# TMElyralab/MuseV

Hardware: NVIDIA H100
Metric: denoised frames/sec at 512x512, 16-frame window, 20 DDIM steps (higher is better)
Workload: dtype f16 (fp32 accumulate)

## Files before the change

musev_b200/csrc/conv_gemm.cu:

```cuda
#include "conv_gemm.cuh"

#include <dlfcn.h>
#include <stdio.h>
#include <stdlib.h>
#include <string.h>

#include <mutex>

#include "ptx.cuh"
#include "stats.cuh"

namespace mvb {

static constexpr int kMaxStages = 8;
static constexpr int kBlockM = 128;
static constexpr int kBlockK = 64;
static constexpr int kABytes = kBlockM * kBlockK * 2;
static constexpr int kSmemBytes = 227 * 1024;
constexpr bool inline_epilogue(int bn) { return bn == 256; }
constexpr int conv_threads(int bn) { return inline_epilogue(bn) ? 384 : 512; }
static constexpr int kMaxStagedN = 160;
static constexpr int kStagingBytes = kBlockM * kMaxStagedN * 4;
static constexpr int kAccLd = 132;
static constexpr int kAccBytes = 2 * 64 * kAccLd * 4;
constexpr int epi_buf_bytes(int bn) { return inline_epilogue(bn) ? kAccBytes : kStagingBytes; }
constexpr int bias_buf_bytes(int bn) { return inline_epilogue(bn) ? 2 * 256 * 4 : kMaxStagedN * 4; }
constexpr int ring_bytes(int bn) { return kSmemBytes - epi_buf_bytes(bn) - bias_buf_bytes(bn) - 1024  - 256 ; }
constexpr int ring_stage_bytes(int bn) { return kABytes + (bn * kBlockK * 2 + 1023) / 1024 * 1024; }
constexpr int ring_stages(int bn) {
  return ring_bytes(bn) / ring_stage_bytes(bn) < kMaxStages ? ring_bytes(bn) / ring_stage_bytes(bn) : kMaxStages;
}
static_assert(ring_stages(64) == 6 && ring_stages(128) == 4 && ring_stages(160) == 4 && ring_stages(256) == 3,
              "shared-memory budget per tile width");
__device__ __forceinline__ float gelu_erf(float x) { return 0.5f * x * (1.f + erff(x * 0.70710678118654752440f)); }
__device__ __forceinline__ float silu(float x) { return __fdividef(x, 1.f + __expf(-x)); }
__device__ __forceinline__ float gelu_fast(float x) {
  const float z = fabsf(x) * 0.70710678118654752440f;
  const float t = __frcp_rn(fmaf(0.3275911f, z, 1.f));
  float poly = fmaf(1.061405429f, t, -1.453152027f);
  poly = fmaf(poly, t, 1.421413741f);
  poly = fmaf(poly, t, -0.284496736f);
  poly = fmaf(poly, t, 0.254829592f);
  poly *= t;
  float e;
  asm("ex2.approx.ftz.f32 %0, %1;" : "=f"(e) : "f"(-z * z * 1.4426950408889634f));
  const float erf_abs = fmaf(-poly, e, 1.f);
  const float erf_v = copysignf(erf_abs, x);
  return 0.5f * x * (1.f + erf_v);
}

__device__ __forceinline__ float rcp_approx(float x) {
  float y;
  asm("rcp.approx.ftz.f32 %0, %1;" : "=f"(y) : "f"(x));
  return y;
}
__device__ __forceinline__ F2 geglu2(F2 val, F2 gate) {
  float g0, g1;
  f2_get(gate, g0, g1);
  const F2 u = f2_make(fabsf(g0), fabsf(g1));
  float d0, d1;
  f2_get(f2_fma(u, f2_make(0.231641888f, 0.231641888f), f2_make(1.f, 1.f)), d0, d1);
  const F2 t = f2_make(rcp_approx(d0), rcp_approx(d1));
  F2 poly = f2_fma(t, f2_make(-0.5307027145f, -0.5307027145f), f2_make(0.7265760135f, 0.7265760135f));
  poly = f2_fma(poly, t, f2_make(-0.7107068705f, -0.7107068705f));
  poly = f2_fma(poly, t, f2_make(0.142248368f, 0.142248368f));
  poly = f2_fma(poly, t, f2_make(-0.127414796f, -0.127414796f));
  poly = f2_mul(poly, t);
  float a0, a1;
  f2_get(f2_mul(f2_mul(u, f2_make(-0.72134752044f, -0.72134752044f)), u), a0, a1);
  float e0, e1;
  asm("ex2.approx.ftz.f32 %0, %1;" : "=f"(e0) : "f"(a0));
  asm("ex2.approx.ftz.f32 %0, %1;" : "=f"(e1) : "f"(a1));
  const F2 gelu = f2_fma(u, f2_mul(poly, f2_make(e0, e1)), f2_make(fmaxf(g0, 0.f), fmaxf(g1, 0.f)));
  return f2_mul(val, gelu);
}

enum : int {
  kEpiGeneric = 0,
  kEpiPlain = 1,
  kEpiResidual = 2,
  kEpiGeglu = 3,
  kEpiAct = 4
};
__device__ __forceinline__ float gelu_act(float x, int act) {
  return act == 2 ? gelu_erf(x) : act == 3 ? __fdividef(x, 1.f + __expf(-1.702f * x)) : x;
}

struct AMaps {
  CUtensorMap m[4];
};

template <int kEpi, class Ld>
__device__ __forceinline__ void finish_run(const ConvGemmParams& p, const Ld& ld32, int c0, int ncol0, const float* sbias,
                                           const float* radd, const uint4 (&rcur)[4], bool row_ok, bool use_res,
                                           long long m, __half* out_row) {
  if constexpr (kEpi != kEpiGeneric && kEpi != kEpiAct) {
    const int nbase = ncol0 + c0;
    uint32_t v[32], vg[32];
    ld32(c0, v);
    if constexpr (kEpi == kEpiGeglu) ld32(c0 + 32, vg);
    if (nbase < p.N && row_ok) {
      const F2 alpha2 = f2_make(p.alpha, p.alpha);
      const float* cbias = sbias + c0;
      const int oc = (kEpi == kEpiGeglu) ? nbase / 2 : nbase;
#pragma unroll
      for (int g = 0; g < 4; ++g) {
        uint32_t o[4];
        if constexpr (kEpi == kEpiGeglu) {
          const uint32_t* vv = (g < 2) ? v : vg;
          const int j0 = (g & 1) * 8;
#pragma unroll
          for (int e = 0; e < 4; ++e) {
            const int j = j0 + 2 * e;
            const float2 bv = *reinterpret_cast<const float2*>(cbias + (g >> 1) * 32 + j);
            const float2 bg = *reinterpret_cast<const float2*>(cbias + (g >> 1) * 32 + 16 + j);
            const F2 val = f2_add(f2_make(__uint_as_float(vv[j]), __uint_as_float(vv[j + 1])), f2_make(bv.x, bv.y));
            const F2 gat = f2_add(f2_make(__uint_as_float(vv[16 + j]), __uint_as_float(vv[16 + j + 1])),
                                  f2_make(bg.x, bg.y));
            float x0, x1;
            f2_get(geglu2(val, gat), x0, x1);
            const __half2 h2 = __floats2half2_rn(x0, x1);
            o[e] = *reinterpret_cast<const uint32_t*>(&h2);
          }
        } else {
          float4 b0 = *reinterpret_cast<const float4*>(cbias + 8 * g);
          float4 b1 = *reinterpret_cast<const float4*>(cbias + 8 * g + 4);
          if (radd) {
            const float4 a0 = __ldg(reinterpret_cast<const float4*>(radd + nbase) + 2 * g);
            const float4 a1 = __ldg(reinterpret_cast<const float4*>(radd + nbase) + 2 * g + 1);
            b0.x += a0.x; b0.y += a0.y; b0.z += a0.z; b0.w += a0.w;
            b1.x += a1.x; b1.y += a1.y; b1.z += a1.z; b1.w += a1.w;
          }
          const float bb[8] = {b0.x, b0.y, b0.z, b0.w, b1.x, b1.y, b1.z, b1.w};
          const __half2* rh2 = reinterpret_cast<const __half2*>(&rcur[g]);
#pragma unroll
          for (int e = 0; e < 4; ++e) {
            const int j = g * 8 + 2 * e;
            F2 x = f2_add(f2_make(__uint_as_float(v[j]), __uint_as_float(v[j + 1])), f2_make(bb[2 * e], bb[2 * e + 1]));
            if constexpr (kEpi == kEpiResidual) {
              const float2 rr = __half22float2(rh2[e]);
              x = f2_fma(x, alpha2, f2_make(rr.x, rr.y));
            }
            float x0, x1;
            f2_get(x, x0, x1);
            const __half2 h2 = __floats2half2_rn(x0, x1);
            o[e] = *reinterpret_cast<const uint32_t*>(&h2);
          }
        }
        *reinterpret_cast<uint4*>(out_row + oc + 8 * g) = make_uint4(o[0], o[1], o[2], o[3]);
      }
    }
  } else {
    float f[32];
    const int nbase = ncol0 + c0;
    if (p.geglu) {
      uint32_t va[32], vb[32];
      ld32(c0, va);
      ld32(c0 + 32, vb);
#pragma unroll
      for (int hsel = 0; hsel < 2; ++hsel) {
        const uint32_t* v = hsel ? vb : va;
        const int nb = nbase + hsel * 32;
#pragma unroll
        for (int j4 = 0; j4 < 4; ++j4) {
          const bool bok = p.bias && nb < p.N;
          const float4 bv = bok ? __ldg(reinterpret_cast<const float4*>(p.bias + nb) + j4) : make_float4(0, 0, 0, 0);
          const float4 bg = bok ? __ldg(reinterpret_cast<const float4*>(p.bias + nb + 16) + j4) : make_float4(0, 0, 0, 0);
          const int j = j4 * 4;
          const F2 v01 = f2_add(f2_make(__uint_as_float(v[j]), __uint_as_float(v[j + 1])), f2_make(bv.x, bv.y));
          const F2 v23 = f2_add(f2_make(__uint_as_float(v[j + 2]), __uint_as_float(v[j + 3])), f2_make(bv.z, bv.w));
          const F2 g01 = f2_add(f2_make(__uint_as_float(v[16 + j]), __uint_as_float(v[16 + j + 1])), f2_make(bg.x, bg.y));
          const F2 g23 = f2_add(f2_make(__uint_as_float(v[16 + j + 2]), __uint_as_float(v[16 + j + 3])), f2_make(bg.z, bg.w));
          f2_get(geglu2(v01, g01), f[hsel * 16 + j], f[hsel * 16 + j + 1]);
          f2_get(geglu2(v23, g23), f[hsel * 16 + j + 2], f[hsel * 16 + j + 3]);
        }
      }
    } else {
      uint32_t v[32];
      ld32(c0, v);
      if (nbase + 32 <= p.N) {
#pragma unroll
        for (int g = 0; g < 8; ++g) {
          float4 b = p.bias ? __ldg(reinterpret_cast<const float4*>(p.bias + nbase) + g) : make_float4(0, 0, 0, 0);
          if (radd) {
            const float4 a4 = __ldg(reinterpret_cast<const float4*>(radd + nbase) + g);
            b.x += a4.x; b.y += a4.y; b.z += a4.z; b.w += a4.w;
          }
          f[g * 4 + 0] = __uint_as_float(v[g * 4 + 0]) + b.x;
          f[g * 4 + 1] = __uint_as_float(v[g * 4 + 1]) + b.y;
          f[g * 4 + 2] = __uint_as_float(v[g * 4 + 2]) + b.z;
          f[g * 4 + 3] = __uint_as_float(v[g * 4 + 3]) + b.w;
        }
      } else {
#pragma unroll
        for (int j = 0; j < 32; ++j) {
          const int nn = nbase + j;
          float x = __uint_as_float(v[j]);
          if (nn < p.N) {
            if (p.bias) x += __ldg(p.bias + nn);
            if (radd) x += __ldg(radd + nn);
          }
          f[j] = x;
        }
      }
    }
    if (row_ok) {
      if (p.out_f32) {
#pragma unroll
        for (int g = 0; g < 8; ++g) {
          const int nn = nbase + g * 4;
          if (nn < p.N) {
            float4 o4;
            o4.x = f[g * 4 + 0] * p.alpha; o4.y = f[g * 4 + 1] * p.alpha;
            o4.z = f[g * 4 + 2] * p.alpha; o4.w = f[g * 4 + 3] * p.alpha;
            if (p.act == 1) { o4.x = silu(o4.x); o4.y = silu(o4.y); o4.z = silu(o4.z); o4.w = silu(o4.w); }
            if constexpr (kEpi == kEpiAct) {
              o4.x = gelu_act(o4.x, p.act); o4.y = gelu_act(o4.y, p.act);
              o4.z = gelu_act(o4.z, p.act); o4.w = gelu_act(o4.w, p.act);
            }
            *reinterpret_cast<float4*>(reinterpret_cast<float*>(p.out) + m * p.ldc + nn) = o4;
          }
        }
      } else {
        const int oc = p.geglu ? nbase / 2 : nbase;
        const int ncols = p.geglu ? p.N / 2 : p.N;
#pragma unroll
        for (int g = 0; g < 4; ++g) {
          if (oc + 8 * g >= ncols) continue;
          __align__(16) __half o[8];
          const __half* rh8 = reinterpret_cast<const __half*>(&rcur[g]);
#pragma unroll
          for (int j = 0; j < 8; ++j) {
            float x = f[g * 8 + j];
            if (!p.geglu) {
              x *= p.alpha;
              if (use_res) x = fmaf(p.beta, __half2float(rh8[j]), x);
              if (p.act == 1) x = silu(x);
              if constexpr (kEpi == kEpiAct) x = gelu_act(x, p.act);
            }
            o[j] = __float2half_rn(x);
          }
          *reinterpret_cast<uint4*>(out_row + oc + 8 * g) = *reinterpret_cast<const uint4*>(o);
        }
      }
    }
  }
}

template <int kEpi, int BN>
__device__ __forceinline__ void inline_epilogue_tile(const ConvGemmParams& p, const float (&acc)[BN / 2], float* sacc,
                                                     float* sbias, int unit, int wg, int t) {
  const int lane = t & 31;
  const int wq = t >> 5;
  const int row_local = t & 63;
  const int half = t >> 6;
  const int r = 64 * wg + row_local;
  float* acc_slice = sacc + wg * 64 * kAccLd;
  float* wbias = sbias + wg * 256;
  const bool use_res = (p.res != nullptr) && !p.geglu && !p.out_f32;
  const int acc_step = p.geglu ? 64 : 32;
  const int nt = unit % p.tiles_nn;
  const int mt = unit / p.tiles_nn;
  const int tw = mt % p.tiles_w;
  const int th = (mt / p.tiles_w) % p.tiles_h;
  const int tn = mt / (p.tiles_w * p.tiles_h);
  const int ncol0 = nt * BN;
  const int rw = r % p.bw;
  const int rh = (r / p.bw) % p.bh;
  const int rn = r / (p.bw * p.bh);
  const int w = tw * p.bw + rw, h = th * p.bh + rh, n = tn * p.bn + rn;
  const bool row_ok = (w < p.W) && (h < p.H) && (n < p.NF);
  const long long m = ((long long)n * p.H + h) * p.W + w;
  const float* radd = (p.rowadd && row_ok) ? p.rowadd + (long long)(m / p.rows_per_group) * p.ld_rowadd : nullptr;
  const __half* res_row = use_res ? p.res + m * p.ld_res : nullptr;
  __half* out_row = reinterpret_cast<__half*>(p.out) + m * p.ldc;

  uint4 rcur[4] = {};
  auto load_res = [&](int c0) {
    if (!use_res || !row_ok) return;
#pragma unroll
    for (int g = 0; g < 4; ++g) {
      const int nn = ncol0 + c0 + g * 8;
      if (c0 + g * 8 < BN && nn < p.N) rcur[g] = __ldg(reinterpret_cast<const uint4*>(res_row + nn));
    }
  };
  named_bar_sync(1 + wg, 128);
  if constexpr (kEpi != kEpiGeneric && kEpi != kEpiAct) {
    for (int c = t; c < BN; c += 128) wbias[c] = (p.bias && ncol0 + c < p.N) ? __ldg(p.bias + ncol0 + c) : 0.f;
  }
#pragma unroll
  for (int u = 0; u < (BN + 127) / 128; ++u) {
    if (u > 0) named_bar_sync(1 + wg, 128);
#pragma unroll
    for (int i = 16 * u; i < 16 * u + 16 && i < BN / 8; ++i) {
      const int rr = 16 * wq + (lane >> 2);
      const int cc = 8 * (i - 16 * u) + 2 * (lane & 3);
      *reinterpret_cast<float2*>(acc_slice + rr * kAccLd + cc) = make_float2(acc[4 * i], acc[4 * i + 1]);
      *reinterpret_cast<float2*>(acc_slice + (rr + 8) * kAccLd + cc) = make_float2(acc[4 * i + 2], acc[4 * i + 3]);
    }
    named_bar_sync(1 + wg, 128);
    const int cend = (128 * u + 128 < BN) ? 128 * u + 128 : BN;
    for (int c0 = 128 * u + half * acc_step; c0 < cend; c0 += 2 * acc_step) {
      const float* srow = acc_slice + row_local * kAccLd - 128 * u;
      auto ld32 = [&](int col, uint32_t (&v)[32]) {
#pragma unroll
        for (int k = 0; k < 8; ++k) {
          const float4 x = *reinterpret_cast<const float4*>(srow + col + 4 * k);
          v[4 * k] = __float_as_uint(x.x); v[4 * k + 1] = __float_as_uint(x.y);
          v[4 * k + 2] = __float_as_uint(x.z); v[4 * k + 3] = __float_as_uint(x.w);
        }
      };
      load_res(c0);
      finish_run<kEpi>(p, ld32, c0, ncol0, wbias, radd, rcur, row_ok, use_res, m, out_row);
    }
  }
}

template <int kEpi, int BN>
__global__ void __launch_bounds__(conv_threads(BN), 1)
conv_gemm_kernel(const __grid_constant__ AMaps tmA, const __grid_constant__ CUtensorMap tmB,
                 const __grid_constant__ ConvGemmParams p) {
  constexpr bool kInline = inline_epilogue(BN);
  static_assert(BN % 32 == 0 && (BN <= kMaxStagedN || kInline), "the staging swizzle and the epilogue take whole 32-column runs");
  constexpr int kProducerRegs = 40, kConsumerRegs = kInline ? 232 : 152, kEpilogueRegs = kInline ? 0 : 168;
  static_assert(128 * (kProducerRegs + kEpilogueRegs) + 256 * kConsumerRegs <= 65536,
                "setmaxnreg split exceeds the register file");
  constexpr int kRingBytes = ring_bytes(BN);
  extern __shared__ uint8_t smem_raw[];
  uint8_t* smem = reinterpret_cast<uint8_t*>((reinterpret_cast<uintptr_t>(smem_raw) + 1023) & ~uintptr_t(1023));
  float* stg = reinterpret_cast<float*>(smem + kRingBytes);
  float* sbias = reinterpret_cast<float*>(smem + kRingBytes + epi_buf_bytes(BN));
  uint64_t* bars = reinterpret_cast<uint64_t*>(smem + kRingBytes + epi_buf_bytes(BN) + bias_buf_bytes(BN));
  uint64_t* full = bars;
  uint64_t* empty = bars + kMaxStages;
  uint64_t* acc_full = bars + 2 * kMaxStages;
  uint64_t* acc_empty = acc_full + 1;
  const int nstages = p.nstages;
  const int stage_bytes = p.stage_bytes;

  const int warp = threadIdx.x >> 5;
  const int lane = threadIdx.x & 31;

  if (threadIdx.x == 0) {
    tma_prefetch_desc(&tmA.m[0]);
    tma_prefetch_desc(&tmA.m[1]);
    tma_prefetch_desc(&tmA.m[2]);
    tma_prefetch_desc(&tmA.m[3]);
    tma_prefetch_desc(&tmB);
    for (int s = 0; s < kMaxStages; ++s) {
      mbar_init(&full[s], 1);
      mbar_init(&empty[s], 8);
    }
    mbar_init(acc_full, 8);
    mbar_init(acc_empty, 4);
    fence_barrier_init();
  }
  __syncthreads();

  const int kb_per_tap = p.kb0 + p.kb1;
  const int num_kb = p.ntaps * kb_per_tap;
  const int tiles_m = p.tiles_w * p.tiles_h * p.tiles_n;
  const int num_units = tiles_m * p.tiles_nn;
  const uint32_t stage_tx = kABytes + (uint32_t)BN * kBlockK * 2;

  if (warp < 4) {
    setmaxnreg_dec<kProducerRegs>();
    if (warp == 0) {
      int stage = 0;
      uint32_t phase = 0;
      for (int unit = blockIdx.x; unit < num_units; unit += gridDim.x) {
        const int nt = unit % p.tiles_nn;
        const int mt = unit / p.tiles_nn;
        const int tw = mt % p.tiles_w;
        const int th = (mt / p.tiles_w) % p.tiles_h;
        const int tn = mt / (p.tiles_w * p.tiles_h);
        const int w0 = tw * p.bw, h0 = th * p.bh, n0 = tn * p.bn;
        int kcol = 0;
        const int ncoord = nt * BN;
        for (int tap = 0; tap < p.ntaps; ++tap) {
          const int xw = w0 + p.dx[tap], yh = h0 + p.dy[tap];
          const int src0 = p.tap_src[tap];
          for (int cb = 0; cb < kb_per_tap; ++cb, kcol += kBlockK) {
            const bool first = cb < p.kb0;
            const int src = src0 + (first ? 0 : 1);
            const int c0 = (first ? cb : cb - p.kb0) * kBlockK;
            const CUtensorMap* tm = &tmA.m[src];
            mbar_wait(&empty[stage], phase ^ 1);
            if (elect_one()) {
              uint8_t* sa = smem + stage * stage_bytes;
              uint8_t* sb = sa + kABytes;
              mbar_expect_tx(&full[stage], stage_tx);
              tma_load_4d(sa, tm, &full[stage], c0, xw, yh, n0);
              tma_load_2d(sb, &tmB, &full[stage], kcol, ncoord);
            }
            __syncwarp();
            if (++stage == nstages) { stage = 0; phase ^= 1; }
          }
        }
      }
    }
    return;
  }

  if (!kInline && warp >= 12) {
    setmaxnreg_inc<kEpilogueRegs>();
    const int r = threadIdx.x - 384;
    const float* srow = stg + r * BN;
    const int sw = r & 7;
    const bool use_res = (p.res != nullptr) && !p.geglu && !p.out_f32;
    const int acc_step = p.geglu ? 64 : 32;
    uint32_t acc_phase = 0;
    for (int unit = blockIdx.x; unit < num_units; unit += gridDim.x) {
      const int nt = unit % p.tiles_nn;
      const int mt = unit / p.tiles_nn;
      const int tw = mt % p.tiles_w;
      const int th = (mt / p.tiles_w) % p.tiles_h;
      const int tn = mt / (p.tiles_w * p.tiles_h);
      const int ncol0 = nt * BN;
      const int rw = r % p.bw;
      const int rh = (r / p.bw) % p.bh;
      const int rn = r / (p.bw * p.bh);
      const int w = tw * p.bw + rw, h = th * p.bh + rh, n = tn * p.bn + rn;
      const bool row_ok = (w < p.W) && (h < p.H) && (n < p.NF);
      const long long m = ((long long)n * p.H + h) * p.W + w;
      const float* radd = (p.rowadd && row_ok) ? p.rowadd + (long long)(m / p.rows_per_group) * p.ld_rowadd : nullptr;
      const __half* res_row = use_res ? p.res + m * p.ld_res : nullptr;
      __half* out_row = reinterpret_cast<__half*>(p.out) + m * p.ldc;

      uint4 rcur[4] = {}, rnext[4] = {};
      auto load_res = [&](int c0, uint4 (&dst)[4]) {
        if (!use_res || !row_ok) return;
#pragma unroll
        for (int g = 0; g < 4; ++g) {
          const int nn = ncol0 + c0 + g * 8;
          if (c0 + g * 8 < BN && nn < p.N) dst[g] = __ldg(reinterpret_cast<const uint4*>(res_row + nn));
        }
      };
      if constexpr (kEpi != kEpiGeneric && kEpi != kEpiAct) {
        named_bar_sync(1, 128);
        for (int c = r; c < BN; c += 128) sbias[c] = (p.bias && ncol0 + c < p.N) ? __ldg(p.bias + ncol0 + c) : 0.f;
        named_bar_sync(1, 128);
      }
      load_res(0, rcur);
      mbar_wait(acc_full, acc_phase);
      for (int c0 = 0; c0 < BN; c0 += acc_step) {
        if constexpr (kEpi == kEpiResidual) load_res(c0 + acc_step, rnext);
        else if (c0 > 0) load_res(c0, rcur);
        auto ld32 = [&](int col, uint32_t (&v)[32]) {
#pragma unroll
          for (int k = 0; k < 8; ++k) {
            const float4 x = *reinterpret_cast<const float4*>(srow + col + 4 * (k ^ sw));
            v[4 * k] = __float_as_uint(x.x); v[4 * k + 1] = __float_as_uint(x.y);
            v[4 * k + 2] = __float_as_uint(x.z); v[4 * k + 3] = __float_as_uint(x.w);
          }
        };
        finish_run<kEpi>(p, ld32, c0, ncol0, sbias, radd, rcur, row_ok, use_res, m, out_row);
        if constexpr (kEpi == kEpiResidual) {
#pragma unroll
          for (int g = 0; g < 4; ++g) rcur[g] = rnext[g];
        }
      }
      __syncwarp();
      if (lane == 0) mbar_arrive(acc_empty);
      acc_phase ^= 1;
    }
    return;
  }

  setmaxnreg_inc<kConsumerRegs>();
  const int wg = (warp - 4) >> 2;
  const int t = threadIdx.x - 128 * (1 + wg);
  const int wq = t >> 5;
  const uint64_t desc0_a = make_desc_k_sw128(smem_u32(smem) + (uint32_t)wg * 64 * 128);
  const uint64_t desc0_b = make_desc_k_sw128(smem_u32(smem) + kABytes);
  const uint32_t stage_step = (uint32_t)stage_bytes >> 4;
  float* stg_row = stg + (64 * wg + 16 * wq + (lane >> 2)) * BN;
  int stage = 0;
  uint32_t phase = 0;
  uint32_t acc_phase = 0;
  float acc[BN / 2];

  for (int unit = blockIdx.x; unit < num_units; unit += gridDim.x) {
    int prev_stage = 0;
    for (int kb = 0; kb < num_kb; ++kb) {
      mbar_wait(&full[stage], phase);
      const uint64_t da = desc0_a + (uint64_t)((uint32_t)stage * stage_step);
      const uint64_t db = desc0_b + (uint64_t)((uint32_t)stage * stage_step);
      wgmma_fence();
      fence_regs(acc);
#pragma unroll
      for (int k = 0; k < kBlockK / 16; ++k)
        Wgmma<BN>::ss(acc, da + (uint64_t)(k * 2), db + (uint64_t)(k * 2), (kb | k) != 0);
      wgmma_commit();
      fence_regs(acc);
      if (kb > 0) {
        wgmma_wait<1>();
        fence_regs(acc);
        __syncwarp();
        if (lane == 0) mbar_arrive(&empty[prev_stage]);
      }
      prev_stage = stage;
      if (++stage == nstages) { stage = 0; phase ^= 1; }
    }
    wgmma_wait<0>();
    fence_regs(acc);
    __syncwarp();
    if (lane == 0) mbar_arrive(&empty[prev_stage]);

    if constexpr (kInline) {
      inline_epilogue_tile<kEpi, BN>(p, acc, stg, sbias, unit, wg, t);
    } else {
      mbar_wait(acc_empty, acc_phase ^ 1);
#pragma unroll
      for (int i = 0; i < BN / 8; ++i) {
        const int off = 4 * ((2 * i + ((lane & 3) >> 1)) ^ (lane >> 2)) + 2 * (lane & 1);
        *reinterpret_cast<float2*>(stg_row + off) = make_float2(acc[4 * i], acc[4 * i + 1]);
        *reinterpret_cast<float2*>(stg_row + 8 * BN + off) = make_float2(acc[4 * i + 2], acc[4 * i + 3]);
      }
      __syncwarp();
      if (lane == 0) mbar_arrive(acc_full);
      acc_phase ^= 1;
    }
  }
}

typedef CUresult (*EncodeTiledFn)(CUtensorMap*, CUtensorMapDataType, cuuint32_t, void*, const cuuint64_t*,
                                  const cuuint64_t*, const cuuint32_t*, const cuuint32_t*, CUtensorMapInterleave,
                                  CUtensorMapSwizzle, CUtensorMapL2promotion, CUtensorMapFloatOOBfill);

EncodeTiledFn get_encode_fn() {
  static EncodeTiledFn fn = nullptr;
  static bool tried = false;
  if (!tried) {
    tried = true;
    void* h = dlopen("libcuda.so.1", RTLD_NOW | RTLD_GLOBAL);
    if (!h) h = dlopen("libcuda.so", RTLD_NOW | RTLD_GLOBAL);
    if (h) fn = reinterpret_cast<EncodeTiledFn>(dlsym(h, "cuTensorMapEncodeTiled"));
  }
  return fn;
}

namespace {
struct MapKey {
  uint64_t ptr, d[4], s[3];
  uint32_t box[4], rank, swz;
  bool operator==(const MapKey& o) const { return memcmp(this, &o, sizeof(MapKey)) == 0; }
};
struct MapSlot {
  MapKey key;
  CUtensorMap map;
  bool used;
};
static_assert(sizeof(MapKey) == 88, "MapKey is compared and hashed bytewise: no padding allowed");
static_assert(sizeof(MapSlot) % 64 == 0, "slots keep the 64-byte alignment of CUtensorMap");
constexpr uint32_t kMapSlots = 1u << 14;
std::mutex g_map_mutex;
MapSlot* g_map_slots = nullptr;
uint32_t g_map_count = 0;
unsigned long long g_map_hits = 0, g_map_misses = 0;

uint64_t hash_key(const MapKey& k) {
  const uint64_t* w = reinterpret_cast<const uint64_t*>(&k);
  uint64_t h = 0x9e3779b97f4a7c15ull;
  for (size_t i = 0; i < sizeof(MapKey) / 8; ++i) {
    h ^= w[i] + 0x9e3779b97f4a7c15ull + (h << 6) + (h >> 2);
    h *= 0xff51afd7ed558ccdull;
    h ^= h >> 33;
  }
  return h;
}
bool cache_enabled() {
  static const bool on = !(getenv("MVB_TMAP_CACHE") && atoi(getenv("MVB_TMAP_CACHE")) == 0);
  return on;
}

bool encode_raw(CUtensorMap* m, const MapKey& k) {
  EncodeTiledFn fn = get_encode_fn();
  if (!fn) return false;
  cuuint64_t gd[4] = {k.d[0], k.d[1], k.d[2], k.d[3]};
  cuuint64_t gs[3] = {k.s[0] * 2, k.s[1] * 2, k.s[2] * 2};
  cuuint32_t bx[4] = {k.box[0], k.box[1], k.box[2], k.box[3]};
  cuuint32_t es[4] = {1, 1, 1, 1};
  CUresult r = fn(m, CU_TENSOR_MAP_DATA_TYPE_FLOAT16, k.rank, reinterpret_cast<void*>(k.ptr), gd, gs, bx, es,
                  CU_TENSOR_MAP_INTERLEAVE_NONE, (CUtensorMapSwizzle)k.swz, CU_TENSOR_MAP_L2_PROMOTION_L2_256B,
                  CU_TENSOR_MAP_FLOAT_OOB_FILL_NONE);
  return r == CUDA_SUCCESS;
}

bool encode_cached(CUtensorMap* m, const MapKey& k) {
  if (!cache_enabled()) return encode_raw(m, k);
  std::lock_guard<std::mutex> lock(g_map_mutex);
  if (!g_map_slots) {
    g_map_slots = static_cast<MapSlot*>(aligned_alloc(64, sizeof(MapSlot) * kMapSlots));
    if (g_map_slots) memset(g_map_slots, 0, sizeof(MapSlot) * kMapSlots);
  }
  if (!g_map_slots) return encode_raw(m, k);
  uint32_t i = (uint32_t)hash_key(k) & (kMapSlots - 1);
  while (g_map_slots[i].used) {
    if (g_map_slots[i].key == k) {
      *m = g_map_slots[i].map;
      ++g_map_hits;
      return true;
    }
    i = (i + 1) & (kMapSlots - 1);
  }
  if (!encode_raw(m, k)) return false;
  ++g_map_misses;
  if (g_map_count >= kMapSlots / 4 * 3) {
    memset(g_map_slots, 0, sizeof(MapSlot) * kMapSlots);
    g_map_count = 0;
    i = (uint32_t)hash_key(k) & (kMapSlots - 1);
  }
  g_map_slots[i].key = k;
  g_map_slots[i].map = *m;
  g_map_slots[i].used = true;
  ++g_map_count;
  return true;
}
}

void tensor_map_cache_stats(unsigned long long* hits, unsigned long long* misses) {
  std::lock_guard<std::mutex> lock(g_map_mutex);
  *hits = g_map_hits;
  *misses = g_map_misses;
}

bool encode_map_4d_sw(CUtensorMap* m, const void* ptr, const uint64_t dims[4], const uint64_t strides_elems[3],
                      const uint32_t box[4], CUtensorMapSwizzle swz) {
  MapKey k;
  memset(&k, 0, sizeof(k));
  k.ptr = reinterpret_cast<uint64_t>(ptr);
  for (int i = 0; i < 4; ++i) { k.d[i] = dims[i]; k.box[i] = box[i]; }
  for (int i = 0; i < 3; ++i) k.s[i] = strides_elems[i];
  k.rank = 4;
  k.swz = (uint32_t)swz;
  return encode_cached(m, k);
}
bool encode_map_4d(CUtensorMap* m, const void* ptr, const uint64_t dims[4], const uint64_t strides_elems[3],
                   const uint32_t box[4]) {
  return encode_map_4d_sw(m, ptr, dims, strides_elems, box, CU_TENSOR_MAP_SWIZZLE_128B);
}

bool encode_map_2d(CUtensorMap* m, const void* ptr, uint64_t d0, uint64_t d1, uint64_t stride1_elems, uint32_t b0,
                   uint32_t b1) {
  MapKey k;
  memset(&k, 0, sizeof(k));
  k.ptr = reinterpret_cast<uint64_t>(ptr);
  k.d[0] = d0; k.d[1] = d1;
  k.s[0] = stride1_elems;
  k.box[0] = b0; k.box[1] = b1;
  k.rank = 2;
  k.swz = (uint32_t)CU_TENSOR_MAP_SWIZZLE_128B;
  return encode_cached(m, k);
}

static int ceil_div(int a, int b) { return (a + b - 1) / b; }

static void pick_box(int W, int H, int NF, int* bw, int* bh, int* bn) {
  long long best = -1;
  for (int w = 128; w >= 1; w >>= 1) {
    for (int h = 128 / w; h >= 1; h >>= 1) {
      const int n = 128 / (w * h);
      const long long padded = (long long)ceil_div(W, w) * ceil_div(H, h) * ceil_div(NF, n);
      if (best < 0 || padded < best) {
        best = padded;
        *bw = w; *bh = h; *bn = n;
      }
    }
  }
}

static const int kBlockNs[4] = {64, 128, 160, 256};

static int pick_block_n(int N, int geglu, int gelu, long long tiles_m, int num_sms) {
  int best = 0;
  double best_cost = 1e30;
  for (int i = 3; i >= 0; --i) {
    const int bn = kBlockNs[i];
    if (geglu && (bn % 64)) continue;
    if (gelu && bn == 256) continue;
    const int tn = ceil_div(N, bn);
    const long long tiles = tiles_m * tn;
    const long long waves = (tiles + num_sms - 1) / num_sms;
    const double cost = (double)waves * (bn + 24.0);
    if (cost < best_cost - 1e-9) { best_cost = cost; best = bn; }
  }
  return best;
}

static cudaError_t launch_common(cudaStream_t stream, const CUtensorMap* maps, int nmaps, ConvGemmParams& p,
                                 const __half* wt, long long ktot, const Epilogue& ep, int num_sms, const char** err) {
  typedef void (*KernelFn)(const AMaps, const CUtensorMap, const ConvGemmParams);
#define MVB_GEMM_ROW(BN) \
  {conv_gemm_kernel<kEpiGeneric, BN>, conv_gemm_kernel<kEpiPlain, BN>, conv_gemm_kernel<kEpiResidual, BN>, \
   conv_gemm_kernel<kEpiGeglu, BN>, conv_gemm_kernel<kEpiAct, BN>}
  static const KernelFn kernels[4][5] = {MVB_GEMM_ROW(64), MVB_GEMM_ROW(128), MVB_GEMM_ROW(160),
                                         {conv_gemm_kernel<kEpiGeneric, 256>, conv_gemm_kernel<kEpiPlain, 256>,
                                          conv_gemm_kernel<kEpiResidual, 256>, conv_gemm_kernel<kEpiGeglu, 256>, nullptr}};
#undef MVB_GEMM_ROW
  static bool attr_set_dev[64] = {};
  int cur_dev = 0;
  cudaGetDevice(&cur_dev);
  bool& attr_set = attr_set_dev[cur_dev & 63];
  if (!attr_set) {
    for (int a = 0; a < 4; ++a)
      for (int b = 0; b < 5; ++b) {
        if (!kernels[a][b]) continue;
        cudaError_t e = cudaFuncSetAttribute(reinterpret_cast<const void*>(kernels[a][b]),
                                             cudaFuncAttributeMaxDynamicSharedMemorySize, kSmemBytes);
        if (e != cudaSuccess) { *err = "cudaFuncSetAttribute(conv_gemm_kernel)"; return e; }
      }
    attr_set = true;
  }
  const long long tiles_m = (long long)p.tiles_w * p.tiles_h * p.tiles_n;
  const int gelu = ep.act == 2 || ep.act == 3;
  p.block_n = pick_block_n(p.N, ep.geglu, gelu, tiles_m, num_sms);
  int bn_idx = 0;
  while (kBlockNs[bn_idx] != p.block_n) ++bn_idx;
  p.tiles_nn = ceil_div(p.N, p.block_n);
  p.stage_bytes = ring_stage_bytes(p.block_n);
  p.nstages = ring_stages(p.block_n);
  p.out = ep.out; p.ldc = ep.ldc; p.bias = ep.bias; p.rowadd = ep.rowadd;
  p.rows_per_group = ep.rows_per_group > 0 ? ep.rows_per_group : 1;
  p.ld_rowadd = ep.ld_rowadd; p.res = ep.res; p.ld_res = ep.ld_res; p.alpha = ep.alpha; p.beta = ep.beta;
  p.geglu = ep.geglu; p.act = ep.act; p.out_f32 = ep.out_f32;
  if (ep.out_f32 && (ep.geglu || ep.res)) { *err = "conv_gemm: fp32 output excludes geglu/residual"; return cudaErrorInvalidValue; }
  if ((ep.ldc % (ep.out_f32 ? 4 : 8)) || (reinterpret_cast<uintptr_t>(ep.out) % 16)) {
    *err = "conv_gemm: the output must be 16-byte aligned with a row stride of whole 16-byte vectors";
    return cudaErrorInvalidValue;
  }
  CUtensorMap tmB;
  if (!encode_map_2d(&tmB, wt, (uint64_t)ktot, (uint64_t)p.N, (uint64_t)ktot, 64u, (uint32_t)p.block_n)) {
    *err = "cuTensorMapEncodeTiled(B) failed";
    return cudaErrorInvalidValue;
  }
  const long long num_tiles = tiles_m * p.tiles_nn;
  const int grid = (int)(num_tiles < num_sms ? num_tiles : num_sms);
  int epi = kEpiGeneric;
  if (!ep.out_f32 && ep.act == 0) {
    if (ep.geglu) { if (p.N % 64 == 0 && !ep.rowadd) epi = kEpiGeglu; }
    else if (p.N % 32 == 0) {
      if (ep.res && ep.beta == 1.f) epi = kEpiResidual;
      else if (!ep.res && ep.alpha == 1.f) epi = kEpiPlain;
    }
  }
  if (gelu) epi = kEpiAct;
  static const bool trace = getenv("MVB_TRACE") != nullptr;
  if (trace) {
    char taps[9 * 10 + 1];
    int len = 0;
    for (int i = 0; i < p.ntaps; ++i) len += snprintf(taps + len, sizeof(taps) - len, "%s%d:%d", i ? "," : "", p.dy[i], p.dx[i]);
    int s2 = 0;
    for (int i = 0; i < p.ntaps; ++i) if (p.tap_src[i]) s2 = p.dy[0] < 0 ? 1 : 2;
    fprintf(stderr, "MVB_TRACE gemm M=%lld N=%d K=%lld taps=%d block_n=%d tiles=%lld geglu=%d res=%d f32=%d epi=%d "
            "W=%d H=%d NF=%d c0=%d c1=%d offsets=%s s2=%d bias=%d rowadd=%d rpg=%d alpha=%.9g beta=%.9g act=%d\n",
            (long long)p.W * p.H * p.NF, p.N, ktot, p.ntaps, p.block_n, num_tiles, p.geglu, p.res != nullptr, p.out_f32,
            epi, p.W, p.H, p.NF, p.kb0 * 64, p.kb1 * 64, taps, s2, p.bias != nullptr, p.rowadd != nullptr,
            p.rows_per_group, p.alpha, p.beta, p.act);
  }
  AMaps am;
  for (int i = 0; i < 4; ++i) am.m[i] = maps[i < nmaps ? i : 0];
  ProfScope prof(stream, KC_GEMM);
  kernels[bn_idx][epi]<<<grid, conv_threads(p.block_n), kSmemBytes, stream>>>(am, tmB, p);
  cudaError_t e = cudaGetLastError();
  if (e != cudaSuccess) *err = "conv_gemm_kernel launch";
  return e;
}

cudaError_t launch_conv_gemm(cudaStream_t stream, const ASource& a0, const ASource* a1, int W, int H, int NF,
                             int ntaps, const int8_t* dy, const int8_t* dx, const __half* wt, int N,
                             const Epilogue& ep, int num_sms, const char** err) {
  if ((a0.C % 64) || (a1 && (a1->C % 64)) || (N % 8) || ntaps < 1 || ntaps > 9) {
    *err = "conv_gemm: channels must be multiples of 64, N a multiple of 8, 1..9 taps";
    return cudaErrorInvalidValue;
  }
  ConvGemmParams p{};
  p.W = W; p.H = H; p.NF = NF;
  pick_box(W, H, NF, &p.bw, &p.bh, &p.bn);
  p.tiles_w = ceil_div(W, p.bw); p.tiles_h = ceil_div(H, p.bh); p.tiles_n = ceil_div(NF, p.bn);
  p.ntaps = ntaps;
  for (int i = 0; i < ntaps; ++i) { p.dy[i] = dy[i]; p.dx[i] = dx[i]; p.tap_src[i] = 0; }
  p.kb0 = a0.C / 64;
  p.kb1 = a1 ? a1->C / 64 : 0;
  p.N = N;
  CUtensorMap maps[2];
  const uint32_t box[4] = {64u, (uint32_t)p.bw, (uint32_t)p.bh, (uint32_t)p.bn};
  {
    const uint64_t dims[4] = {(uint64_t)a0.C, (uint64_t)W, (uint64_t)H, (uint64_t)NF};
    const uint64_t st[3] = {(uint64_t)a0.sW, (uint64_t)a0.sH, (uint64_t)a0.sN};
    if (!encode_map_4d(&maps[0], a0.ptr, dims, st, box)) { *err = "cuTensorMapEncodeTiled(A0) failed"; return cudaErrorInvalidValue; }
  }
  if (a1) {
    const uint64_t dims[4] = {(uint64_t)a1->C, (uint64_t)W, (uint64_t)H, (uint64_t)NF};
    const uint64_t st[3] = {(uint64_t)a1->sW, (uint64_t)a1->sH, (uint64_t)a1->sN};
    if (!encode_map_4d(&maps[1], a1->ptr, dims, st, box)) { *err = "cuTensorMapEncodeTiled(A1) failed"; return cudaErrorInvalidValue; }
  }
  const long long ktot = (long long)ntaps * (a0.C + (a1 ? a1->C : 0));
  return launch_common(stream, maps, a1 ? 2 : 1, p, wt, ktot, ep, num_sms, err);
}

cudaError_t launch_conv_s2(cudaStream_t stream, const __half* x, int C, int W, int H, int NF, const __half* wt, int N,
                           const Epilogue& ep, int num_sms, const char** err, int pad_mode) {
  if ((C % 64) || (N % 8) || (W % 2) || (H % 2)) {
    *err = "conv_s2: channels multiple of 64, even H and W";
    return cudaErrorInvalidValue;
  }
  if (pad_mode != 1 && pad_mode != 2) {
    *err = "conv_s2: pad mode must be 1 (pad 1 on every side) or 2 (pad (0, 1, 0, 1))";
    return cudaErrorInvalidValue;
  }
  const int Wo = W / 2, Ho = H / 2;
  ConvGemmParams p{};
  p.W = Wo; p.H = Ho; p.NF = NF;
  pick_box(Wo, Ho, NF, &p.bw, &p.bh, &p.bn);
  p.tiles_w = ceil_div(Wo, p.bw); p.tiles_h = ceil_div(Ho, p.bh); p.tiles_n = ceil_div(NF, p.bn);
  p.ntaps = 9;
  static const int8_t kPhase[2][3] = {{1, 0, 1}, {0, 1, 0}}, kOff[2][3] = {{-1, 0, 0}, {0, 0, 1}};
  const int m = pad_mode - 1;
  for (int ky = 0; ky < 3; ++ky)
    for (int kx = 0; kx < 3; ++kx) {
      const int i = ky * 3 + kx;
      p.dy[i] = kOff[m][ky];
      p.dx[i] = kOff[m][kx];
      p.tap_src[i] = (int8_t)(kPhase[m][ky] * 2 + kPhase[m][kx]);
    }
  p.kb0 = C / 64; p.kb1 = 0; p.N = N;
  CUtensorMap maps[4];
  const uint32_t box[4] = {64u, (uint32_t)p.bw, (uint32_t)p.bh, (uint32_t)p.bn};
  for (int py = 0; py < 2; ++py)
    for (int px = 0; px < 2; ++px) {
      const uint64_t dims[4] = {(uint64_t)C, (uint64_t)Wo, (uint64_t)Ho, (uint64_t)NF};
      const uint64_t st[3] = {(uint64_t)2 * C, (uint64_t)2 * W * C, (uint64_t)H * W * C};
      if (!encode_map_4d(&maps[py * 2 + px], x + ((long long)py * W + px) * C, dims, st, box)) {
        *err = "cuTensorMapEncodeTiled(phase) failed";
        return cudaErrorInvalidValue;
      }
    }
  return launch_common(stream, maps, 4, p, wt, 9LL * C, ep, num_sms, err);
}

}
```

Baseline: 5.391.

## Move conv GEMM epilogue stores and residual loads to TMA with swizzled run staging

The epilogue warpgroup now writes each 32-column output run into swizzled shared memory and issues a 4D TMA store, instead of per-thread global stores. For residual epilogues, a producer warp streams the residual tiles through a small TMA-fed shared ring, replacing per-thread __ldg loads. The staging layout changes to 32-column run blocks, and the pipeline stage counts now depend on the epilogue kind, so plain epilogues gain stages while residual ones may lose one. This adds named barriers and proxy fences per run, and requires the output and residual tensors to tile cleanly by the spatial box.

```diff
diff --git a/musev_b200/csrc/conv_gemm.cu b/musev_b200/csrc/conv_gemm.cu
--- a/musev_b200/csrc/conv_gemm.cu
+++ b/musev_b200/csrc/conv_gemm.cu
@@ -20,17 +20,35 @@
 constexpr bool inline_epilogue(int bn) { return bn == 256; }
 constexpr int conv_threads(int bn) { return inline_epilogue(bn) ? 384 : 512; }
 static constexpr int kMaxStagedN = 160;
-static constexpr int kStagingBytes = kBlockM * kMaxStagedN * 4;
+static constexpr int kRunFloats = kBlockM * 32;
+static constexpr int kRunBytes = kBlockM * 32 * 2;
+static constexpr int kResSlots = 4;
 static constexpr int kAccLd = 132;
 static constexpr int kAccBytes = 2 * 64 * kAccLd * 4;
-constexpr int epi_buf_bytes(int bn) { return inline_epilogue(bn) ? kAccBytes : kStagingBytes; }
+
+enum : int {
+  kEpiGeneric = 0,
+  kEpiPlain = 1,
+  kEpiResidual = 2,
+  kEpiGeglu = 3,
+  kEpiAct = 4
+};
+constexpr bool tma_epilogue(int epi, int bn) {
+  return !inline_epilogue(bn) && (epi == kEpiPlain || epi == kEpiResidual || epi == kEpiGeglu);
+}
+constexpr int epi_buf_bytes(int bn) { return inline_epilogue(bn) ? kAccBytes : kBlockM * bn * 4; }
+constexpr int res_ring_bytes(int epi, int bn) { return tma_epilogue(epi, bn) && epi == kEpiResidual ? kResSlots * kRunBytes : 0; }
 constexpr int bias_buf_bytes(int bn) { return inline_epilogue(bn) ? 2 * 256 * 4 : kMaxStagedN * 4; }
-constexpr int ring_bytes(int bn) { return kSmemBytes - epi_buf_bytes(bn) - bias_buf_bytes(bn) - 1024  - 256 ; }
+constexpr int ring_bytes(int epi, int bn) {
+  return kSmemBytes - epi_buf_bytes(bn) - res_ring_bytes(epi, bn) - bias_buf_bytes(bn) - 1024  - 256 ;
+}
 constexpr int ring_stage_bytes(int bn) { return kABytes + (bn * kBlockK * 2 + 1023) / 1024 * 1024; }
-constexpr int ring_stages(int bn) {
-  return ring_bytes(bn) / ring_stage_bytes(bn) < kMaxStages ? ring_bytes(bn) / ring_stage_bytes(bn) : kMaxStages;
-}
-static_assert(ring_stages(64) == 6 && ring_stages(128) == 4 && ring_stages(160) == 4 && ring_stages(256) == 3,
+constexpr int ring_stages(int epi, int bn) {
+  return ring_bytes(epi, bn) / ring_stage_bytes(bn) < kMaxStages ? ring_bytes(epi, bn) / ring_stage_bytes(bn) : kMaxStages;
+}
+static_assert(ring_stages(kEpiPlain, 64) == 8 && ring_stages(kEpiPlain, 128) == 5 && ring_stages(kEpiPlain, 160) == 4 &&
+              ring_stages(kEpiResidual, 64) == 6 && ring_stages(kEpiResidual, 128) == 4 &&
+              ring_stages(kEpiResidual, 160) == 3 && ring_stages(kEpiResidual, 256) == 3,
               "shared-memory budget per tile width");
 __device__ __forceinline__ float gelu_erf(float x) { return 0.5f * x * (1.f + erff(x * 0.70710678118654752440f)); }
 __device__ __forceinline__ float silu(float x) { return __fdividef(x, 1.f + __expf(-x)); }
@@ -75,13 +93,6 @@
   return f2_mul(val, gelu);
 }
 
-enum : int {
-  kEpiGeneric = 0,
-  kEpiPlain = 1,
-  kEpiResidual = 2,
-  kEpiGeglu = 3,
-  kEpiAct = 4
-};
 __device__ __forceinline__ float gelu_act(float x, int act) {
   return act == 2 ? gelu_erf(x) : act == 3 ? __fdividef(x, 1.f + __expf(-1.702f * x)) : x;
 }
@@ -89,16 +100,21 @@
 struct AMaps {
   CUtensorMap m[4];
 };
-
-template <int kEpi, class Ld>
-__device__ __forceinline__ void finish_run(const ConvGemmParams& p, const Ld& ld32, int c0, int ncol0, const float* sbias,
-                                           const float* radd, const uint4 (&rcur)[4], bool row_ok, bool use_res,
-                                           long long m, __half* out_row) {
+struct EpiMaps {
+  CUtensorMap out, res;
+};
+
+template <int kEpi, class Ld, class Loaded, class St>
+__device__ __forceinline__ void finish_run(const ConvGemmParams& p, const Ld& ld32, const Loaded& loaded, const St& st16,
+                                           int c0, int ncol0, const float* sbias, const float* radd,
+                                           const uint4 (&rcur)[4], bool row_ok, bool use_res, long long m,
+                                           __half* out_row) {
   if constexpr (kEpi != kEpiGeneric && kEpi != kEpiAct) {
     const int nbase = ncol0 + c0;
     uint32_t v[32], vg[32];
     ld32(c0, v);
     if constexpr (kEpi == kEpiGeglu) ld32(c0 + 32, vg);
+    loaded();
     if (nbase < p.N && row_ok) {
       const F2 alpha2 = f2_make(p.alpha, p.alpha);
       const float* cbias = sbias + c0;
@@ -147,7 +163,7 @@
             o[e] = *reinterpret_cast<const uint32_t*>(&h2);
           }
         }
-        *reinterpret_cast<uint4*>(out_row + oc + 8 * g) = make_uint4(o[0], o[1], o[2], o[3]);
+        st16(oc + 8 * g, g, make_uint4(o[0], o[1], o[2], o[3]));
       }
     }
   } else {
@@ -311,7 +327,8 @@
         }
       };
       load_res(c0);
-      finish_run<kEpi>(p, ld32, c0, ncol0, wbias, radd, rcur, row_ok, use_res, m, out_row);
+      finish_run<kEpi>(p, ld32, [] {}, [&](int col, int, uint4 o) { *reinterpret_cast<uint4*>(out_row + col) = o; },
+                       c0, ncol0, wbias, radd, rcur, row_ok, use_res, m, out_row);
     }
   }
 }
@@ -319,22 +336,30 @@
 template <int kEpi, int BN>
 __global__ void __launch_bounds__(conv_threads(BN), 1)
 conv_gemm_kernel(const __grid_constant__ AMaps tmA, const __grid_constant__ CUtensorMap tmB,
-                 const __grid_constant__ ConvGemmParams p) {
+                 const __grid_constant__ EpiMaps tmE, const __grid_constant__ ConvGemmParams p) {
   constexpr bool kInline = inline_epilogue(BN);
+  constexpr bool kTma = tma_epilogue(kEpi, BN);
+  constexpr bool kResRing = res_ring_bytes(kEpi, BN) > 0;
   static_assert(BN % 32 == 0 && (BN <= kMaxStagedN || kInline), "the staging swizzle and the epilogue take whole 32-column runs");
   constexpr int kProducerRegs = 40, kConsumerRegs = kInline ? 232 : 152, kEpilogueRegs = kInline ? 0 : 168;
   static_assert(128 * (kProducerRegs + kEpilogueRegs) + 256 * kConsumerRegs <= 65536,
                 "setmaxnreg split exceeds the register file");
-  constexpr int kRingBytes = ring_bytes(BN);
+  constexpr int kRingEnd = ring_stages(kEpi, BN) * ring_stage_bytes(BN);
+  static_assert(kRingEnd % 1024 == 0 && kRingEnd + epi_buf_bytes(BN) + res_ring_bytes(kEpi, BN) + bias_buf_bytes(BN) + 256 + 1024 <=
+                kSmemBytes, "shared-memory layout");
   extern __shared__ uint8_t smem_raw[];
   uint8_t* smem = reinterpret_cast<uint8_t*>((reinterpret_cast<uintptr_t>(smem_raw) + 1023) & ~uintptr_t(1023));
-  float* stg = reinterpret_cast<float*>(smem + kRingBytes);
-  float* sbias = reinterpret_cast<float*>(smem + kRingBytes + epi_buf_bytes(BN));
-  uint64_t* bars = reinterpret_cast<uint64_t*>(smem + kRingBytes + epi_buf_bytes(BN) + bias_buf_bytes(BN));
+  float* stg = reinterpret_cast<float*>(smem + kRingEnd);
+  uint8_t* sres = smem + kRingEnd + epi_buf_bytes(BN);
+  float* sbias = reinterpret_cast<float*>(sres + res_ring_bytes(kEpi, BN));
+  uint64_t* bars = reinterpret_cast<uint64_t*>(sres + res_ring_bytes(kEpi, BN) + bias_buf_bytes(BN));
   uint64_t* full = bars;
   uint64_t* empty = bars + kMaxStages;
   uint64_t* acc_full = bars + 2 * kMaxStages;
   uint64_t* acc_empty = acc_full + 1;
+  uint64_t* res_full = acc_full + 2;
+  uint64_t* res_empty = res_full + kResSlots;
+  static_assert(2 * kMaxStages + 2 + 2 * kResSlots <= 256 / 8, "barrier area");
   const int nstages = p.nstages;
   const int stage_bytes = p.stage_bytes;
 
@@ -347,12 +372,18 @@
     tma_prefetch_desc(&tmA.m[2]);
     tma_prefetch_desc(&tmA.m[3]);
     tma_prefetch_desc(&tmB);
+    if constexpr (kTma) tma_prefetch_desc(&tmE.out);
+    if constexpr (kResRing) tma_prefetch_desc(&tmE.res);
     for (int s = 0; s < kMaxStages; ++s) {
       mbar_init(&full[s], 1);
       mbar_init(&empty[s], 8);
     }
     mbar_init(acc_full, 8);
     mbar_init(acc_empty, 4);
+    for (int s = 0; s < kResSlots; ++s) {
+      mbar_init(&res_full[s], 1);
+      mbar_init(&res_empty[s], 1);
+    }
     fence_barrier_init();
   }
   __syncthreads();
@@ -398,6 +429,26 @@
           }
         }
       }
+    } else if (kResRing && warp == 1) {
+      int slot = 0;
+      uint32_t phase = 0;
+      for (int unit = blockIdx.x; unit < num_units; unit += gridDim.x) {
+        const int nt = unit % p.tiles_nn;
+        const int mt = unit / p.tiles_nn;
+        const int tw = mt % p.tiles_w;
+        const int th = (mt / p.tiles_w) % p.tiles_h;
+        const int tn = mt / (p.tiles_w * p.tiles_h);
+        const int ncol0 = nt * BN;
+        for (int c0 = 0; c0 < BN && ncol0 + c0 < p.N; c0 += 32) {
+          mbar_wait(&res_empty[slot], phase ^ 1);
+          if (elect_one()) {
+            mbar_expect_tx(&res_full[slot], kRunBytes);
+            tma_load_4d(sres + slot * kRunBytes, &tmE.res, &res_full[slot], ncol0 + c0, tw * p.bw, th * p.bh, tn * p.bn);
+          }
+          __syncwarp();
+          if (++slot == kResSlots) { slot = 0; phase ^= 1; }
+        }
+      }
     }
     return;
   }
@@ -405,11 +456,14 @@
   if (!kInline && warp >= 12) {
     setmaxnreg_inc<kEpilogueRegs>();
     const int r = threadIdx.x - 384;
-    const float* srow = stg + r * BN;
+    const float* srow = stg + r * 32;
     const int sw = r & 7;
+    const int sw64 = (r >> 1) & 3;
     const bool use_res = (p.res != nullptr) && !p.geglu && !p.out_f32;
     const int acc_step = p.geglu ? 64 : 32;
     uint32_t acc_phase = 0;
+    int rslot = 0;
+    uint32_t rphase = 0;
     for (int unit = blockIdx.x; unit < num_units; unit += gridDim.x) {
       const int nt = unit % p.tiles_nn;
       const int mt = unit / p.tiles_nn;
@@ -427,13 +481,13 @@
       const __half* res_row = use_res ? p.res + m * p.ld_res : nullptr;
       __half* out_row = reinterpret_cast<__half*>(p.out) + m * p.ldc;
 
-      uint4 rcur[4] = {}, rnext[4] = {};
-      auto load_res = [&](int c0, uint4 (&dst)[4]) {
+      uint4 rcur[4] = {};
+      auto load_res = [&](int c0) {
         if (!use_res || !row_ok) return;
 #pragma unroll
         for (int g = 0; g < 4; ++g) {
           const int nn = ncol0 + c0 + g * 8;
-          if (c0 + g * 8 < BN && nn < p.N) dst[g] = __ldg(reinterpret_cast<const uint4*>(res_row + nn));
+          if (c0 + g * 8 < BN && nn < p.N) rcur[g] = __ldg(reinterpret_cast<const uint4*>(res_row + nn));
         }
       };
       if constexpr (kEpi != kEpiGeneric && kEpi != kEpiAct) {
@@ -441,29 +495,52 @@
         for (int c = r; c < BN; c += 128) sbias[c] = (p.bias && ncol0 + c < p.N) ? __ldg(p.bias + ncol0 + c) : 0.f;
         named_bar_sync(1, 128);
       }
-      load_res(0, rcur);
+      if constexpr (!kTma) load_res(0);
       mbar_wait(acc_full, acc_phase);
       for (int c0 = 0; c0 < BN; c0 += acc_step) {
-        if constexpr (kEpi == kEpiResidual) load_res(c0 + acc_step, rnext);
-        else if (c0 > 0) load_res(c0, rcur);
         auto ld32 = [&](int col, uint32_t (&v)[32]) {
 #pragma unroll
           for (int k = 0; k < 8; ++k) {
-            const float4 x = *reinterpret_cast<const float4*>(srow + col + 4 * (k ^ sw));
+            const float4 x = *reinterpret_cast<const float4*>(srow + (col >> 5) * kRunFloats + 4 * (k ^ sw));
             v[4 * k] = __float_as_uint(x.x); v[4 * k + 1] = __float_as_uint(x.y);
             v[4 * k + 2] = __float_as_uint(x.z); v[4 * k + 3] = __float_as_uint(x.w);
           }
         };
-        finish_run<kEpi>(p, ld32, c0, ncol0, sbias, radd, rcur, row_ok, use_res, m, out_row);
-        if constexpr (kEpi == kEpiResidual) {
-#pragma unroll
-          for (int g = 0; g < 4; ++g) rcur[g] = rnext[g];
-        }
-      }
+        if constexpr (kTma) {
+          if (ncol0 + c0 >= p.N) break;
+          if constexpr (kEpi == kEpiResidual) {
+            mbar_wait(&res_full[rslot], rphase);
+            const uint4* rrow = reinterpret_cast<const uint4*>(sres + rslot * kRunBytes + r * 64);
+#pragma unroll
+            for (int g = 0; g < 4; ++g) rcur[g] = rrow[g ^ sw64];
+          }
+          uint8_t* orun = reinterpret_cast<uint8_t*>(stg) + (c0 >> 5) * (kRunFloats * 4);
+          finish_run<kEpi>(p, ld32, [] { named_bar_sync(1, 128); },
+                           [&](int, int g, uint4 o) { *reinterpret_cast<uint4*>(orun + r * 64 + 16 * (g ^ sw64)) = o; },
+                           c0, ncol0, sbias, radd, rcur, row_ok, use_res, m, out_row);
+          fence_proxy_async();
+          named_bar_sync(1, 128);
+          if (r == 0) {
+            if constexpr (kEpi == kEpiResidual) mbar_arrive(&res_empty[rslot]);
+            tma_store_4d(&tmE.out, orun, kEpi == kEpiGeglu ? (ncol0 + c0) / 2 : ncol0 + c0, tw * p.bw, th * p.bh,
+                         tn * p.bn);
+            tma_store_commit();
+          }
+          if constexpr (kEpi == kEpiResidual) {
+            if (++rslot == kResSlots) { rslot = 0; rphase ^= 1; }
+          }
+        } else {
+          if (c0 > 0) load_res(c0);
+          finish_run<kEpi>(p, ld32, [] {}, [&](int col, int, uint4 o) { *reinterpret_cast<uint4*>(out_row + col) = o; },
+                           c0, ncol0, sbias, radd, rcur, row_ok, use_res, m, out_row);
+        }
+      }
+      if (kTma && r == 0) tma_store_wait_read<0>();
       __syncwarp();
       if (lane == 0) mbar_arrive(acc_empty);
       acc_phase ^= 1;
     }
+    if (kTma && r == 0) tma_store_wait_all();
     return;
   }
 
@@ -474,7 +551,7 @@
   const uint64_t desc0_a = make_desc_k_sw128(smem_u32(smem) + (uint32_t)wg * 64 * 128);
   const uint64_t desc0_b = make_desc_k_sw128(smem_u32(smem) + kABytes);
   const uint32_t stage_step = (uint32_t)stage_bytes >> 4;
-  float* stg_row = stg + (64 * wg + 16 * wq + (lane >> 2)) * BN;
+  float* stg_row = stg + (64 * wg + 16 * wq + (lane >> 2)) * 32;
   int stage = 0;
   uint32_t phase = 0;
   uint32_t acc_phase = 0;
@@ -513,9 +590,9 @@
       mbar_wait(acc_empty, acc_phase ^ 1);
 #pragma unroll
       for (int i = 0; i < BN / 8; ++i) {
-        const int off = 4 * ((2 * i + ((lane & 3) >> 1)) ^ (lane >> 2)) + 2 * (lane & 1);
+        const int off = (i >> 2) * kRunFloats + 4 * ((2 * (i & 3) + ((lane & 3) >> 1)) ^ (lane >> 2)) + 2 * (lane & 1);
         *reinterpret_cast<float2*>(stg_row + off) = make_float2(acc[4 * i], acc[4 * i + 1]);
-        *reinterpret_cast<float2*>(stg_row + 8 * BN + off) = make_float2(acc[4 * i + 2], acc[4 * i + 3]);
+        *reinterpret_cast<float2*>(stg_row + 8 * 32 + off) = make_float2(acc[4 * i + 2], acc[4 * i + 3]);
       }
       __syncwarp();
       if (lane == 0) mbar_arrive(acc_full);
@@ -690,7 +767,7 @@
 
 static cudaError_t launch_common(cudaStream_t stream, const CUtensorMap* maps, int nmaps, ConvGemmParams& p,
                                  const __half* wt, long long ktot, const Epilogue& ep, int num_sms, const char** err) {
-  typedef void (*KernelFn)(const AMaps, const CUtensorMap, const ConvGemmParams);
+  typedef void (*KernelFn)(const AMaps, const CUtensorMap, const EpiMaps, const ConvGemmParams);
 #define MVB_GEMM_ROW(BN) \
   {conv_gemm_kernel<kEpiGeneric, BN>, conv_gemm_kernel<kEpiPlain, BN>, conv_gemm_kernel<kEpiResidual, BN>, \
    conv_gemm_kernel<kEpiGeglu, BN>, conv_gemm_kernel<kEpiAct, BN>}
@@ -718,8 +795,6 @@
   int bn_idx = 0;
   while (kBlockNs[bn_idx] != p.block_n) ++bn_idx;
   p.tiles_nn = ceil_div(p.N, p.block_n);
-  p.stage_bytes = ring_stage_bytes(p.block_n);
-  p.nstages = ring_stages(p.block_n);
   p.out = ep.out; p.ldc = ep.ldc; p.bias = ep.bias; p.rowadd = ep.rowadd;
   p.rows_per_group = ep.rows_per_group > 0 ? ep.rows_per_group : 1;
   p.ld_rowadd = ep.ld_rowadd; p.res = ep.res; p.ld_res = ep.ld_res; p.alpha = ep.alpha; p.beta = ep.beta;
@@ -729,6 +804,10 @@
     *err = "conv_gemm: the output must be 16-byte aligned with a row stride of whole 16-byte vectors";
     return cudaErrorInvalidValue;
   }
+  if (ep.res && ((ep.ld_res % 8) || (reinterpret_cast<uintptr_t>(ep.res) % 16))) {
+    *err = "conv_gemm: the residual must be 16-byte aligned with a row stride of whole 16-byte vectors";
+    return cudaErrorInvalidValue;
+  }
   CUtensorMap tmB;
   if (!encode_map_2d(&tmB, wt, (uint64_t)ktot, (uint64_t)p.N, (uint64_t)ktot, 64u, (uint32_t)p.block_n)) {
     *err = "cuTensorMapEncodeTiled(B) failed";
@@ -745,6 +824,29 @@
     }
   }
   if (gelu) epi = kEpiAct;
+  p.stage_bytes = ring_stage_bytes(p.block_n);
+  p.nstages = ring_stages(epi, p.block_n);
+  const bool tma_epi = tma_epilogue(epi, p.block_n);
+  EpiMaps em;
+  memset(&em, 0, sizeof(em));
+  if (tma_epi) {
+    const uint32_t box[4] = {32u, (uint32_t)p.bw, (uint32_t)p.bh, (uint32_t)p.bn};
+    const uint64_t ncols = (uint64_t)(ep.geglu ? p.N / 2 : p.N);
+    const uint64_t od[4] = {ncols, (uint64_t)p.W, (uint64_t)p.H, (uint64_t)p.NF};
+    const uint64_t os[3] = {(uint64_t)ep.ldc, (uint64_t)ep.ldc * p.W, (uint64_t)ep.ldc * p.W * p.H};
+    if (!encode_map_4d_sw(&em.out, ep.out, od, os, box, CU_TENSOR_MAP_SWIZZLE_64B)) {
+      *err = "cuTensorMapEncodeTiled(out) failed";
+      return cudaErrorInvalidValue;
+    }
+    if (epi == kEpiResidual) {
+      const uint64_t rd[4] = {(uint64_t)p.N, (uint64_t)p.W, (uint64_t)p.H, (uint64_t)p.NF};
+      const uint64_t rs[3] = {(uint64_t)ep.ld_res, (uint64_t)ep.ld_res * p.W, (uint64_t)ep.ld_res * p.W * p.H};
+      if (!encode_map_4d_sw(&em.res, ep.res, rd, rs, box, CU_TENSOR_MAP_SWIZZLE_64B)) {
+        *err = "cuTensorMapEncodeTiled(residual) failed";
+        return cudaErrorInvalidValue;
+      }
+    }
+  }
   static const bool trace = getenv("MVB_TRACE") != nullptr;
   if (trace) {
     char taps[9 * 10 + 1];
@@ -753,15 +855,15 @@
     int s2 = 0;
     for (int i = 0; i < p.ntaps; ++i) if (p.tap_src[i]) s2 = p.dy[0] < 0 ? 1 : 2;
     fprintf(stderr, "MVB_TRACE gemm M=%lld N=%d K=%lld taps=%d block_n=%d tiles=%lld geglu=%d res=%d f32=%d epi=%d "
-            "W=%d H=%d NF=%d c0=%d c1=%d offsets=%s s2=%d bias=%d rowadd=%d rpg=%d alpha=%.9g beta=%.9g act=%d\n",
+            "epi_io=%s W=%d H=%d NF=%d c0=%d c1=%d offsets=%s s2=%d bias=%d rowadd=%d rpg=%d alpha=%.9g beta=%.9g act=%d\n",
             (long long)p.W * p.H * p.NF, p.N, ktot, p.ntaps, p.block_n, num_tiles, p.geglu, p.res != nullptr, p.out_f32,
-            epi, p.W, p.H, p.NF, p.kb0 * 64, p.kb1 * 64, taps, s2, p.bias != nullptr, p.rowadd != nullptr,
+            epi, tma_epi ? "tma" : "lsu", p.W, p.H, p.NF, p.kb0 * 64, p.kb1 * 64, taps, s2, p.bias != nullptr, p.rowadd != nullptr,
             p.rows_per_group, p.alpha, p.beta, p.act);
   }
   AMaps am;
   for (int i = 0; i < 4; ++i) am.m[i] = maps[i < nmaps ? i : 0];
   ProfScope prof(stream, KC_GEMM);
-  kernels[bn_idx][epi]<<<grid, conv_threads(p.block_n), kSmemBytes, stream>>>(am, tmB, p);
+  kernels[bn_idx][epi]<<<grid, conv_threads(p.block_n), kSmemBytes, stream>>>(am, tmB, em, p);
   cudaError_t e = cudaGetLastError();
   if (e != cudaSuccess) *err = "conv_gemm_kernel launch";
   return e;
```

Result: faster. 5.668, median of 6 (+5.1%).
